# zqqqqz2000/MixGRPO

Hardware: AMD Instinct MI355X
Metric: GRPO train-step images/sec, FLUX.1-dev 1024^2 (higher is better)
Workload: dtype bf16

## Files before the change

mixgrpo_amd/csrc/small.hip:

```cpp
#include "../../include/mixgrpo_hip.h"
#include "common.h"

namespace {

__global__ void __launch_bounds__(256) skinny_linear_kernel(const bf16_raw* __restrict__ x, long ldx,
                                                            const bf16_raw* __restrict__ W, long ldw,
                                                            const bf16_raw* __restrict__ bias,
                                                            bf16_raw* __restrict__ out, long ldo, int Bn, int N, int K) {
  __shared__ f32x4 red[3][64];
  const int lane = threadIdx.x & 63, w = threadIdx.x >> 6;
  const int n0 = blockIdx.x * 16;
  const int fr = lane & 15, fq = lane >> 4;
  int nrow = n0 + fr;
  if (nrow >= N) nrow = N - 1;
  int brow = fr < Bn ? fr : Bn - 1;
  const int kchunk = ((K / 32 + 3) / 4) * 32;
  const int kbeg = min(w * kchunk, K), kend = min(kbeg + kchunk, K);
  const bf16_raw* wp = W + (long)nrow * ldw + fq * 8;
  const bf16_raw* xp = x + (long)brow * ldx + fq * 8;
  f32x4 acc = {0.f, 0.f, 0.f, 0.f};
  int k = kbeg;
  for (; k + 128 <= kend; k += 128) {
    s16x8 a0 = *reinterpret_cast<const s16x8*>(wp + k), a1 = *reinterpret_cast<const s16x8*>(wp + k + 32);
    s16x8 a2 = *reinterpret_cast<const s16x8*>(wp + k + 64), a3 = *reinterpret_cast<const s16x8*>(wp + k + 96);
    s16x8 b0 = *reinterpret_cast<const s16x8*>(xp + k), b1 = *reinterpret_cast<const s16x8*>(xp + k + 32);
    s16x8 b2 = *reinterpret_cast<const s16x8*>(xp + k + 64), b3 = *reinterpret_cast<const s16x8*>(xp + k + 96);
    acc = __builtin_amdgcn_mfma_f32_16x16x32_bf16(a0, b0, acc, 0, 0, 0);
    acc = __builtin_amdgcn_mfma_f32_16x16x32_bf16(a1, b1, acc, 0, 0, 0);
    acc = __builtin_amdgcn_mfma_f32_16x16x32_bf16(a2, b2, acc, 0, 0, 0);
    acc = __builtin_amdgcn_mfma_f32_16x16x32_bf16(a3, b3, acc, 0, 0, 0);
  }
  for (; k < kend; k += 32) {
    s16x8 a0 = *reinterpret_cast<const s16x8*>(wp + k);
    s16x8 b0 = *reinterpret_cast<const s16x8*>(xp + k);
    acc = __builtin_amdgcn_mfma_f32_16x16x32_bf16(a0, b0, acc, 0, 0, 0);
  }
  if (w > 0) red[w - 1][lane] = acc;
  __syncthreads();
  if (w > 0) return;
#pragma unroll
  for (int i = 0; i < 3; ++i) {
    const f32x4 o = red[i][lane];
    acc[0] += o[0]; acc[1] += o[1]; acc[2] += o[2]; acc[3] += o[3];
  }
  if (fr < Bn) {
#pragma unroll
    for (int r = 0; r < 4; ++r) {
      const int n = n0 + 4 * fq + r;
      if (n < N) {
        float v = acc[r];
        if (bias) v += bf2f(bias[n]);
        out[(long)fr * ldo + n] = f2bf(v);
      }
    }
  }
}

__global__ void __launch_bounds__(256) skinny_wgrad_kernel(const bf16_raw* __restrict__ dout, long ldd,
                                                           const bf16_raw* __restrict__ x, long ldx,
                                                           float* __restrict__ dW, long ldw, float* __restrict__ dbias,
                                                           int Bn, int N, int K) {
  const int n = blockIdx.y;
  float dn[16];
  float sb = 0.f;
#pragma unroll
  for (int b = 0; b < 16; ++b) {
    dn[b] = b < Bn ? bf2f(dout[(long)b * ldd + n]) : 0.f;
    sb += dn[b];
  }
  if (dbias && blockIdx.x == 0 && threadIdx.x == 0) dbias[n] += sb;
  for (int k = (blockIdx.x * 256 + threadIdx.x) * 4; k < K; k += gridDim.x * 256 * 4) {
    float4 g = *reinterpret_cast<float4*>(dW + (long)n * ldw + k);
    for (int b = 0; b < Bn; ++b) {
      const uint2 u = *reinterpret_cast<const uint2*>(x + (long)b * ldx + k);
      g.x += dn[b] * bf2f(u.x & 0xffff); g.y += dn[b] * bf2f(u.x >> 16);
      g.z += dn[b] * bf2f(u.y & 0xffff); g.w += dn[b] * bf2f(u.y >> 16);
    }
    *reinterpret_cast<float4*>(dW + (long)n * ldw + k) = g;
  }
}

constexpr int SD_G = 128;
__global__ void __launch_bounds__(256) skinny_dgrad_kernel(const bf16_raw* __restrict__ dout, long ldd,
                                                           const bf16_raw* __restrict__ W, long ldw, float* __restrict__ part,
                                                           int Bn, int N, int K) {
  extern __shared__ float dsh[];
  const int g = blockIdx.y;
  const int nrows = (N - g + SD_G - 1) / SD_G;
  for (int id = threadIdx.x; id < nrows * 8; id += 256) {
    const int i = id >> 3, b = id & 7;
    dsh[id] = b < Bn ? bf2f(dout[(long)b * ldd + g + (long)i * SD_G]) : 0.f;
  }
  __syncthreads();
  const int c = (blockIdx.x * 256 + threadIdx.x) * 8;
  if (c >= K) return;
  float acc[8][8];
#pragma unroll
  for (int b = 0; b < 8; ++b)
#pragma unroll
    for (int e = 0; e < 8; ++e) acc[b][e] = 0.f;
  const bf16_raw* wp = W + (long)g * ldw + c;
  const long step = (long)SD_G * ldw;
  int i = 0;
  for (; i + 4 <= nrows; i += 4) {
    uint4 u[4];
// ... 84 lines not shown
    a.x = bf2f(u.x & 0xffff) * scale; a.y = bf2f(u.x >> 16) * scale; a.z = bf2f(u.y & 0xffff) * scale; a.w = bf2f(u.y >> 16) * scale;
    b.x = bf2f(u.z & 0xffff) * scale; b.y = bf2f(u.z >> 16) * scale; b.z = bf2f(u.w & 0xffff) * scale; b.w = bf2f(u.w >> 16) * scale;
    *reinterpret_cast<float4*>(y + i) = a;
    *reinterpret_cast<float4*>(y + i + 4) = b;
  }
}

constexpr int GR_ROWS = 64;
__global__ void __launch_bounds__(256) gate_bwd_kernel(const bf16_raw* __restrict__ dout, long ldd, long d_rpb,
                                                       long d_bstride, const bf16_raw* __restrict__ y, long ldy,
                                                       const bf16_raw* __restrict__ gate, long gate_ld,
                                                       bf16_raw* __restrict__ dy, long lddy, float* __restrict__ part,
                                                       long rows_per_batch, int D, int blocks_per_batch) {
  const long b = blockIdx.y / blocks_per_batch;
  const long r0 = (long)(blockIdx.y % blocks_per_batch) * GR_ROWS;
  const int c = (blockIdx.x * 256 + threadIdx.x) * 2;
  if (c >= D) return;
  const uint32_t gu = *reinterpret_cast<const uint32_t*>(gate + b * gate_ld + c);
  const float g0 = bf2f(gu & 0xffff), g1 = bf2f(gu >> 16);
  float a0 = 0.f, a1 = 0.f;
  const long rend = min(r0 + (long)GR_ROWS, rows_per_batch);
  for (long r = r0; r < rend; ++r) {
    const long m = b * rows_per_batch + r;
    const uint32_t du = *reinterpret_cast<const uint32_t*>(dout + b * d_bstride + r * ldd + c);
    const uint32_t yu = *reinterpret_cast<const uint32_t*>(y + m * ldy + c);
    const float d0 = bf2f(du & 0xffff), d1 = bf2f(du >> 16);
    a0 += d0 * bf2f(yu & 0xffff);
    a1 += d1 * bf2f(yu >> 16);
    *reinterpret_cast<uint32_t*>(dy + m * lddy + c) = (uint32_t)f2bf(g0 * d0) | ((uint32_t)f2bf(g1 * d1) << 16);
  }
  part[(long)blockIdx.y * D + c] = a0;
  part[(long)blockIdx.y * D + c + 1] = a1;
}

__global__ void __launch_bounds__(256) gate_bwd_finish_kernel(const float* __restrict__ part, bf16_raw* __restrict__ dgate,
                                                              long gate_ld, int D, int blocks_per_batch) {
  __shared__ float red[4][64];
  const int b = blockIdx.y;
  const int cx = threadIdx.x & 63, ky = threadIdx.x >> 6;
  const int c = blockIdx.x * 64 + cx;
  float s = 0.f;
  if (c < D)
    for (int k = ky; k < blocks_per_batch; k += 4) s += part[((long)b * blocks_per_batch + k) * D + c];
  red[ky][cx] = s;
  __syncthreads();
  if (ky == 0 && c < D) dgate[(long)b * gate_ld + c] = f2bf((red[0][cx] + red[1][cx]) + (red[2][cx] + red[3][cx]));
}

}

extern "C" int mgx_skinny_linear(const uint16_t* x, long ldx, const uint16_t* W, long ldw, const uint16_t* bias,
                                 uint16_t* out, long ldo, int Bn, int N, int K, void* stream) {
  MGX_REQUIRE(x && W && out, "null operand");
  MGX_REQUIRE(Bn >= 1 && Bn <= 16, "skinny linear handles 1..16 rows");
  MGX_REQUIRE(K % 32 == 0 && ldx % 8 == 0 && ldw % 8 == 0, "K must be a multiple of 32 with 16-byte aligned rows");
  skinny_linear_kernel<<<cdiv(N, 16), 256, 0, (hipStream_t)stream>>>(x, ldx, W, ldw, bias, out, ldo, Bn, N, K);
  MGX_CHECK_LAUNCH();
  return MGX_OK;
}

extern "C" int mgx_skinny_wgrad(const uint16_t* dout, long ldd, const uint16_t* x, long ldx, float* dW, long ldw,
                                float* dbias, int Bn, int N, int K, void* stream) {
  MGX_REQUIRE(dout && x && dW, "null operand");
  MGX_REQUIRE(Bn >= 1 && Bn <= 16, "skinny wgrad handles 1..16 rows");
  MGX_REQUIRE(K % 4 == 0 && ldx % 4 == 0 && ldw % 4 == 0, "K must be a multiple of 4");
  int gx = cdiv(K, 1024);
  skinny_wgrad_kernel<<<dim3(gx, N), 256, 0, (hipStream_t)stream>>>(dout, ldd, x, ldx, dW, ldw, dbias, Bn, N, K);
  MGX_CHECK_LAUNCH();
  return MGX_OK;
}

extern "C" long mgx_skinny_dgrad_workspace(int Bn, int K) { return (long)SD_G * (Bn < 8 ? Bn : 8) * K; }

extern "C" int mgx_skinny_dgrad(const uint16_t* dout, long ldd, const uint16_t* W, long ldw, uint16_t* dx, long lddx,
                                float* ws, int Bn, int N, int K, int accumulate, void* stream) {
  MGX_REQUIRE(dout && W && dx && ws, "null operand");
  MGX_REQUIRE(Bn >= 1 && Bn <= 8, "skinny dgrad handles 1..8 rows per call");
  MGX_REQUIRE(N >= SD_G && K % 8 == 0 && ldw % 8 == 0 && ((uintptr_t)W % 16 == 0), "weight rows must be 16-byte addressable");
  hipStream_t st = (hipStream_t)stream;
  const size_t lds = (size_t)cdiv(N, SD_G) * 8 * sizeof(float);
  MGX_REQUIRE(lds <= 65536, "too many weight rows");
  skinny_dgrad_kernel<<<dim3(cdiv(K, 2048), SD_G), 256, lds, st>>>(dout, ldd, W, ldw, ws, Bn, N, K);
  skinny_dgrad_finish_kernel<<<cdiv((long)Bn * K, 256), 256, 0, st>>>(ws, dx, lddx, Bn, K, accumulate);
  MGX_CHECK_LAUNCH();
  return MGX_OK;
}

extern "C" int mgx_ew_bf16(const uint16_t* a, const uint16_t* b, uint16_t* y, long n, int op, void* stream) {
  MGX_REQUIRE(a && y && n > 0 && op >= 0 && op <= 3, "bad argument");
  MGX_REQUIRE(op == 0 || op == 3 || b, "binary op needs b");
  int nb = cdiv(n, 256);
  if (nb > 2048) nb = 2048;
  ew_kernel<<<nb, 256, 0, (hipStream_t)stream>>>(a, b, y, n, op);
  MGX_CHECK_LAUNCH();
  return MGX_OK;
}

extern "C" int mgx_sincos_embed(const float* t, uint16_t* out, int Bn, void* stream) {
  MGX_REQUIRE(t && out && Bn > 0, "bad argument");
  sincos_embed_kernel<<<Bn, 128, 0, (hipStream_t)stream>>>(t, out, Bn);
  MGX_CHECK_LAUNCH();
  return MGX_OK;
}

extern "C" int mgx_cast_f32_bf16(const float* x, uint16_t* y, long n, void* stream) {
  MGX_REQUIRE(x && y && n > 0 && n % 4 == 0, "bad argument");
  int nb = cdiv(n, 1024);
  if (nb > 4096) nb = 4096;
  cast_f32_bf16_kernel<<<nb, 256, 0, (hipStream_t)stream>>>(x, y, n);
// ... 32 lines not shown
```

mixgrpo_amd/flux.py:

```python
import json
import math
import os
from dataclasses import asdict, dataclass
from typing import Dict, List, Tuple

import torch

from . import ops
from ._lib import MgxError
from .ops import BF16, F32, Rows, EPI_BIAS, EPI_BIAS_GELU, EPI_BIAS_GATE_RES


@dataclass
class FluxConfig:
    patch_size: int = 1
    in_channels: int = 64
    num_layers: int = 19
    num_single_layers: int = 38
    attention_head_dim: int = 128
    num_attention_heads: int = 24
    joint_attention_dim: int = 4096
    pooled_projection_dim: int = 768
    guidance_embeds: bool = True
    axes_dims_rope: Tuple[int, int, int] = (16, 56, 56)
# ... 166 lines not shown
        self.out = e(B, N, cfg.patch_size * cfg.patch_size * cfg.in_channels)
        self.lse = e(B, H, S, dtype=F32)
        self.train = None
        self._f8 = None
        self._f8_bwd = None
        self._dims = (H, hd)

    def fp8_bwd_workspace(self):
        if self._f8_bwd is None:
            H, _ = self._dims
            dev = self.X.device
            self._f8_bwd = (torch.empty(ops.attn_bwd_fp8_workspace(self.B, H, self.S, self.Sp), dtype=torch.uint8, device=dev),
                            torch.empty(4 * self.B * H, dtype=F32, device=dev))
        return self._f8_bwd

    def fp8_operands(self):
        if self._f8 is None:
            H, hd = self._dims
            u8 = lambda *shape: torch.empty(*shape, dtype=torch.uint8, device=self.X.device)
            self._f8 = (u8(self.B, H, self.S, hd), u8(self.B, H, self.S, hd), u8(self.B, H, hd, self.Sp),
                        torch.empty(3 * self.B * H, dtype=F32, device=self.X.device))
        return self._f8

    def view(self, B, kv_len=None):
        return self if B == self.B and kv_len is None else _WorkView(self, B, kv_len)


class _WorkView:

    def __init__(self, base, B, kv_len=None):
        assert B <= base.B
        self.base, self.B, self.L, self.N, self.S, self.Sp, self.kv_len = base, B, base.L, base.N, base.S, base.Sp, kv_len
        M = B * base.S
        self.X, self.Q, self.K, self.Vt, self.O, self.cat = (t[:B] for t in (base.X, base.Q, base.K, base.Vt, base.O, base.cat))
        self.nrm, self.qkv, self.hid = base.nrm[:M], base.qkv[:M], base.hid[:M]
        self.in16, self.out, self.lse = base.in16[:B * base.N], base.out[:B], base.lse[:B]

    def fp8_operands(self):
        q8, k8, v8t, amax = self.base.fp8_operands()
        return q8[:self.B], k8[:self.B], v8t[:self.B], amax

    def fp8_bwd_workspace(self):
        return self.base.fp8_bwd_workspace()

    @property
    def train(self):
        return self.base.train

    @train.setter
    def train(self, v):
        self.base.train = v


class FluxTransformer2DModel(torch.nn.Module):

    def __init__(self, config: FluxConfig = None, device="cuda", attention_dtype="bf16", **cfg_kwargs):
        super().__init__()
        if attention_dtype not in ("bf16", "fp8"):
            raise ValueError(f"attention_dtype {attention_dtype!r} is not supported (bf16 | fp8)")
        self.attention_dtype = attention_dtype
        self.cfg = config or FluxConfig(**cfg_kwargs)
        self.config = self.cfg.to_dict()
        dev = torch.device(device)
        if dev.type != "cuda":
            raise MgxError("FluxTransformer2DModel (mixgrpo_amd) runs on an MI355X only; there is no CPU path")
        self.store = ParamStore(self.cfg, dev)
        self.flat_param = torch.nn.Parameter(self.store.w32, requires_grad=True)
        self._work: Dict[Tuple[int, int], _Work] = {}
        self._rope_cache = {}
        self.recompute = True
        self.last_route = None
        self.padded_kv_calls = 0
        self.last_train_route = None
        self.padded_kv_train_calls = 0

    def state_dict(self, *args, **kwargs):
        return {k: self.store.view(self.store.w32, k) for k in self.store.index}

    def load_state_dict(self, sd, strict=True):
        missing = [k for k in self.store.index if k not in sd]
        unexpected = [k for k in sd if k not in self.store.index]
        if strict and (missing or unexpected):
            raise RuntimeError(f"load_state_dict: missing {missing[:5]} unexpected {unexpected[:5]}")
        with torch.no_grad():
            for k, v in sd.items():
                if k in self.store.index:
                    self.store.view(self.store.w32, k).copy_(v.to(F32))
        self.store.sync_bf16()
        return missing, unexpected

    def init_synthetic(self, seed=0, std=0.02, bias_std=0.0):
        self.store.init_synthetic(seed, std, bias_std)
        return self

    def W(self, name):
        return self.store.view(self.store.w16, name)

    def W32(self, name):
        return self.store.view(self.store.w32, name)

    def clip_grad_norm_(self, max_norm):
        g = self.store.ensure_grad()
        nsq = torch.zeros(1, dtype=F32, device=g.device)
        ops.sqnorm(g, nsq)
        total = nsq.sqrt()
        coef = torch.clamp(max_norm / (total + 1e-6), max=1.0)
# ... 106 lines not shown
            ops.ew(h1, None, a1, 0)
            h2 = torch.empty_like(h1)
            ops.skinny_linear(a1, self.W(f"time_text_embed.{name}.linear_2.weight"),
                              self.W(f"time_text_embed.{name}.linear_2.bias"), h2, d, d)
            if keep is not None:
                keep[name] = (x, h1, a1)
            return h2

        te = torch.empty(B, 256, dtype=BF16, device=dev)
        ops.sincos_embed(t, te)
        temb = mlp("timestep_embedder", te, 256)
        if self.cfg.guidance_embeds:
            ge = torch.empty(B, 256, dtype=BF16, device=dev)
            ops.sincos_embed(gd, ge)
            gemb = mlp("guidance_embedder", ge, 256)
            t2 = torch.empty_like(temb)
            ops.ew(temb, gemb, t2, 2)
            temb = t2
        pe = mlp("text_embedder", pooled.to(BF16).contiguous(), self.cfg.pooled_projection_dim)
        t3 = torch.empty_like(temb)
        ops.ew(temb, pe, t3, 2)
        st = torch.empty_like(t3)
        ops.ew(t3, None, st, 0)
        return t3, st

    def _stream_rows(self, t, w, which, width):
        if which == "txt":
            return Rows(t, w.B * w.L, width, w.L, w.S * width)
        return Rows(t[0, w.L:], w.B * w.N, width, w.N, w.S * width)

    def _streams(self, w):
        streams = (("txt", "norm1_context", ("add_q_proj", "add_k_proj", "add_v_proj"), "norm_added_q", "norm_added_k",
                    "to_add_out", "ff_context", w.L, 0),
                   ("img", "norm1", ("to_q", "to_k", "to_v"), "norm_q", "norm_k", "to_out.0", "ff", w.N, w.L))
        return streams, {"txt": slice(0, w.B * w.L), "img": slice(w.B * w.L, w.B * w.S)}

    def _double_block(self, i, w, st, cos, sin, pl, mods_in=None):
        cfg, d, H = self.cfg, self.cfg.dim, self.cfg.num_attention_heads
        p = f"transformer_blocks.{i}"
        B = w.B
        dev = self.store.device
        mods = {}
        streams, sl = self._streams(w)
        W16, fused = self.W, self.store.fused
        if pl.restore is not None:
            w.X.copy_(pl.restore)
        for name, norm, qkvn, nq, nk, outn, ffn, rows, s0 in streams:
            if mods_in is not None:
                m = mods_in[name]
            else:
                m = torch.empty(B, 6 * d, dtype=BF16, device=dev)
                ops.skinny_linear(st, W16(f"{p}.{norm}.linear.weight"), W16(f"{p}.{norm}.linear.bias"), m, 6 * d, d)
            mods[name] = m
            ops.ln_modulate(self._stream_rows(pl.x_in, w, name, d), m[:, 0:d], m[:, d:2 * d], 6 * d, pl.nrm1[sl[name]], d)
        if pl.fused_qkv:
            for name, _, qkvn, nq, nk, _, _, rows, s0 in streams:
                self._qkv_nograd(pl.nrm1[sl[name]], f"{p}.attn.{qkvn[0]}", pl.qkv[sl[name]], w, rows, s0,
                                 self.W32(f"{p}.attn.{nq}.weight"), self.W32(f"{p}.attn.{nk}.weight"), cos, sin)
        else:
            for name, _, qkvn, *_ in (streams if pl.run_qkv else ()):
                ops.gemm(Rows.of(pl.nrm1[sl[name]]), fused(self.store.w16, f"{p}.attn.{qkvn[0]}.weight", 3 * d),
                         fused(self.store.w16, f"{p}.attn.{qkvn[0]}.bias", 3 * d), Rows.of(pl.qkv[sl[name]]), 3 * d, d)
            for name, norm, qkvn, nq, nk, outn, ffn, rows, s0 in streams:
                ops.qk_norm_rope(pl.qkv[sl[name]], self.W32(f"{p}.attn.{nq}.weight"), self.W32(f"{p}.attn.{nk}.weight"), cos, sin,
                                 w.Q, w.K, w.Vt, B, H, w.S, w.Sp, rows, s0, V=pl.V, Qt=pl.Qt, Kt=pl.Kt, q_scale=self.q_scale())
        if pl.run_attn:
            self._attn(w, pl.O, pl.lse, d, w.S * d)
        part = lambda t, name: None if t is None else t[sl[name]]
        if pl.run_out:
            for name, _, _, _, _, outn, *_ in streams:
                ops.gemm(self._stream_rows(pl.O, w, name, d), W16(f"{p}.attn.{outn}.weight"), W16(f"{p}.attn.{outn}.bias"),
                         self._stream_rows(w.X, w, name, d), d, d, EPI_BIAS_GATE_RES, gate=mods[name][:, 2 * d:3 * d],
                         gate_ld=6 * d, aux=part(pl.y_attn, name))
            if pl.x_mid is not None:
                pl.x_mid.copy_(w.X)
        x_mid = w.X if pl.run_out else pl.x_mid
        for name in ("txt", "img"):
            m = mods[name]
            ops.ln_modulate(self._stream_rows(x_mid, w, name, d), m[:, 3 * d:4 * d], m[:, 4 * d:5 * d], 6 * d, pl.nrm2[sl[name]], d)
        for name, _, _, _, _, _, ffn, *_ in (streams if pl.run_ff else ()):
            ops.gemm(Rows.of(pl.nrm2[sl[name]]), W16(f"{p}.{ffn}.net.0.proj.weight"), W16(f"{p}.{ffn}.net.0.proj.bias"),
                     Rows.of(w.hid[sl[name]]), 4 * d, d, EPI_BIAS_GELU, aux=part(pl.hid_pre, name))
        for name, _, _, _, _, _, ffn, *_ in (streams if pl.run_out else ()):
            ops.gemm(Rows.of(w.hid[sl[name]]), W16(f"{p}.{ffn}.net.2.weight"), W16(f"{p}.{ffn}.net.2.bias"),
                     self._stream_rows(w.X, w, name, d), d, 4 * d, EPI_BIAS_GATE_RES, gate=mods[name][:, 5 * d:6 * d],
                     gate_ld=6 * d, aux=part(pl.y_ff, name))
        return mods

    def _single_block(self, i, w, st, cos, sin, pl, mod_in=None):
        cfg, d, H = self.cfg, self.cfg.dim, self.cfg.num_attention_heads
        p = f"single_transformer_blocks.{i}"
        B, S = w.B, w.S
        M = B * S
        if pl.restore is not None:
            w.X.copy_(pl.restore)
        if mod_in is not None:
            m = mod_in
        else:
            m = torch.empty(B, 3 * d, dtype=BF16, device=self.store.device)
            ops.skinny_linear(st, self.W(f"{p}.norm.linear.weight"), self.W(f"{p}.norm.linear.bias"), m, 3 * d, d)
        Xa = Rows(pl.x_in, M, d, S, S * d)
        ops.ln_modulate(Xa, m[:, 0:d], m[:, d:2 * d], 3 * d, pl.nrm1, d)
        wq, wk = self.W32(f"{p}.attn.norm_q.weight"), self.W32(f"{p}.attn.norm_k.weight")
        if pl.fused_qkv:
            self._qkv_nograd(pl.nrm1, f"{p}.attn.to_q", pl.qkv, w, S, 0, wq, wk, cos, sin)
        elif pl.run_qkv:
            ops.gemm(Rows.of(pl.nrm1), self.store.fused(self.store.w16, f"{p}.attn.to_q.weight", 3 * d),
                     self.store.fused(self.store.w16, f"{p}.attn.to_q.bias", 3 * d), Rows.of(pl.qkv), 3 * d, d)
        cat2 = w.cat.view(M, 5 * d)
        if pl.run_ff:
            ops.gemm(Rows.of(pl.nrm1), self.W(f"{p}.proj_mlp.weight"), self.W(f"{p}.proj_mlp.bias"),
                     Rows(cat2[0, d:], M, 5 * d), 4 * d, d, EPI_BIAS_GELU, aux=pl.hid_pre)
        if not pl.fused_qkv:
            ops.qk_norm_rope(pl.qkv, wq, wk, cos, sin, w.Q, w.K, w.Vt, B, H, S, w.Sp, S, 0, V=pl.V, Qt=pl.Qt, Kt=pl.Kt,
                             q_scale=self.q_scale())
        if pl.run_attn:
            self._attn(w, pl.O, pl.lse, pl.ldo, S * pl.ldo)
            if pl.O_keep is not None:
                pl.O_keep.copy_(w.cat[:, :, :d])
        elif not pl.lean:
            w.cat[:, :, :d].copy_(pl.O_keep)
        if pl.run_out:
            ops.gemm(Rows.of(cat2), self.W(f"{p}.proj_out.weight"), self.W(f"{p}.proj_out.bias"), Xa, d, 5 * d,
                     EPI_BIAS_GATE_RES, gate=m[:, 2 * d:3 * d], gate_ld=3 * d, aux=pl.y_attn)
        return m

    def _embed(self, w, hidden_states, encoder_hidden_states):
        d = self.cfg.dim
        B, N, L = w.B, w.N, w.L
        hs = hidden_states.detach()
        if hs.dtype == BF16:
            w.in16.copy_(hs.reshape(B * N, -1))
        else:
            ops.cast_bf16(hs.to(F32).contiguous().view(-1), w.in16.view(-1))
        ops.gemm(Rows.of(w.in16), self.W("x_embedder.weight"), self.W("x_embedder.bias"),
                 self._stream_rows(w.X, w, "img", d), d, self.cfg.in_channels)
        ehs = encoder_hidden_states.detach().to(BF16).contiguous()
        ops.gemm(Rows.of(ehs.view(B * L, -1)), self.W("context_embedder.weight"), self.W("context_embedder.bias"),
                 self._stream_rows(w.X, w, "txt", d), d, self.cfg.joint_attention_dim)
        return ehs

    def _head(self, w, st):
        d = self.cfg.dim
        B, N = w.B, w.N
        e = torch.empty(B, 2 * d, dtype=BF16, device=self.store.device)
        ops.skinny_linear(st, self.W("norm_out.linear.weight"), self.W("norm_out.linear.bias"), e, 2 * d, d)
        nrm = w.nrm[:B * N]
        ops.ln_modulate(self._stream_rows(w.X, w, "img", d), e[:, d:2 * d], e[:, 0:d], 2 * d, nrm, d)
        cout = self.cfg.patch_size * self.cfg.patch_size * self.cfg.in_channels
        out = torch.empty(B, N, cout, dtype=BF16, device=self.store.device)
        ops.gemm(Rows.of(nrm), self.W("proj_out.weight"), self.W("proj_out.bias"), Rows.of(out.view(B * N, cout)), cout, d)
        return out, e

    def forward(self, hidden_states, encoder_hidden_states, timestep, guidance, txt_ids, pooled_projections, img_ids,
                joint_attention_kwargs=None, return_dict=False):
        if torch.is_grad_enabled() and self.training and self.flat_param.requires_grad:
            from .flux_backward import FluxFunction
            out = FluxFunction.apply(self.flat_param, self, hidden_states, encoder_hidden_states, timestep, guidance,
                                     txt_ids, pooled_projections, img_ids)
            return (out,)
        with torch.no_grad():
            out = self._forward_nograd(hidden_states, encoder_hidden_states, timestep, guidance, txt_ids,
                                       pooled_projections, img_ids)
        return (out,)

    def _pad_kv_rows(self, B, L, N):
        S = L + N
        if not ops.ATTN_PAD_KV or S % 256 == 0 or not ops.Q_PRESCALE or self.attention_dtype != "bf16":
            return None
        d, H = self.cfg.dim, self.cfg.num_attention_heads
        Sa = (S + 255) // 256 * 256
        if not all(ops.attn_fwd_kv_path(B, H, Sa, S, ld, Sa * ld) == 1 for ld in (d, 5 * d)):
            return None
        return Sa - L

    def _pad_kv_rows_train(self, B, L, N):
        N_pad = self._pad_kv_rows(B, L, N)
        if N_pad is None:
            return None
        d, H = self.cfg.dim, self.cfg.num_attention_heads
        Sa = L + N_pad
        if not all(ops.attn_bwd_kv_path(B, H, Sa, L + N, ld, Sa * ld) == 1 for ld in (d, 5 * d)):
            return None
        return N_pad

    def _padded_inputs(self, hidden_states, img_ids, N_pad):
        B, N, C = hidden_states.shape
        hs = hidden_states.new_zeros(B, N_pad, C)
        hs[:, :N] = hidden_states
        key = (id(img_ids), img_ids._version, tuple(img_ids.shape), N_pad)
        hit = self._rope_cache.get("pad_ids")
        if hit is None or hit[0] != key:
            ids = torch.cat([img_ids, img_ids.new_zeros(N_pad - N, img_ids.shape[1])], dim=0)
            hit = (key, ids, img_ids)
            self._rope_cache["pad_ids"] = hit
        return hs, hit[1]

    def _forward_nograd(self, hidden_states, encoder_hidden_states, timestep, guidance, txt_ids, pooled_projections,
                        img_ids, collect=None):
        B, N, _ = hidden_states.shape
        L = encoder_hidden_states.shape[1]
        N_pad = self._pad_kv_rows(B, L, N) if collect is None else None
        if N_pad is not None:
            hs, ids = self._padded_inputs(hidden_states, img_ids, N_pad)
            out = self._forward_nograd_on(self._workspace(B, L, N_pad, kv_len=L + N), hs, encoder_hidden_states, timestep, guidance,
                                          txt_ids, pooled_projections, ids, None)
            self.last_route = "padded_kv"
            self.padded_kv_calls += 1
            return out[:, :N].contiguous()
        self.last_route = "plain"
        return self._forward_nograd_on(self._workspace(B, L, N), hidden_states, encoder_hidden_states, timestep, guidance, txt_ids,
                                       pooled_projections, img_ids, collect)

    def _forward_nograd_on(self, w, hidden_states, encoder_hidden_states, timestep, guidance, txt_ids, pooled_projections,
                           img_ids, collect):
        from .flux_backward import _BlockPlan
        B, L = w.B, w.L
        double, single = _BlockPlan(w, True), _BlockPlan(w, False)
        self._embed(w, hidden_states, encoder_hidden_states)
        temb, st = self._temb(B, timestep.to(self.store.device), guidance, pooled_projections)
        cos, sin = self._rope(txt_ids, img_ids)
        if collect is not None:
            collect.update(temb=temb.clone(), x_embed=w.X[:, L:].clone(), ctx_embed=w.X[:, :L].clone())
        for i in range(self.cfg.num_layers):
            self._double_block(i, w, st, cos, sin, double)
            if collect is not None:
                collect[f"double{i}_h"] = w.X[:, L:].clone()
                collect[f"double{i}_c"] = w.X[:, :L].clone()
        for i in range(self.cfg.num_single_layers):
            self._single_block(i, w, st, cos, sin, single)
            if collect is not None:
                collect[f"single{i}_x"] = w.X.clone()
        out, _ = self._head(w, st)
        return out

    def save_pretrained(self, save_dir):
        from safetensors.torch import save_file
        os.makedirs(save_dir, exist_ok=True)
        sd = {k: v.detach().cpu().contiguous() for k, v in self.state_dict().items()}
        save_file(sd, os.path.join(save_dir, "diffusion_pytorch_model.safetensors"))
        cfg = dict(self.config)
        cfg.pop("dtype", None)
        with open(os.path.join(save_dir, "config.json"), "w") as f:
            json.dump(cfg, f, indent=4)

    @classmethod
    def from_pretrained(cls, path, device="cuda", subfolder=None, torch_dtype=None):
        from safetensors.torch import load_file
        if subfolder and os.path.isdir(os.path.join(path, subfolder)):
            path = os.path.join(path, subfolder)
        with open(os.path.join(path, "config.json")) as f:
            raw = json.load(f)
        keys = {f.name for f in FluxConfig.__dataclass_fields__.values()}
        cfg = FluxConfig(**{k: (tuple(v) if k == "axes_dims_rope" else v) for k, v in raw.items() if k in keys})
        m = cls(cfg, device=device)
        index = os.path.join(path, "diffusion_pytorch_model.safetensors.index.json")
        if os.path.exists(index):
            with open(index) as f:
                shards = sorted(set(json.load(f)["weight_map"].values()))
            sd = {}
            for shard in shards:
                sd.update(load_file(os.path.join(path, shard)))
        else:
            sd = load_file(os.path.join(path, "diffusion_pytorch_model.safetensors"))
        m.load_state_dict(sd)
        return m
```

mixgrpo_amd/ops.py:

```python
import os
from dataclasses import dataclass

import torch

from ._lib import check, lib, ptr, stream

EPI_BIAS, EPI_BIAS_GELU, EPI_BIAS_GATE_RES, EPI_F32_ACC, EPI_DGELU = 0, 1, 2, 3, 4
BF16 = torch.bfloat16
F32 = torch.float32


@dataclass
class Rows:
    t: torch.Tensor
    M: int
    ld: int
    rpb: int = 1 << 40
    bstride: int = 0

    @staticmethod
    def of(t):
        cols = t.shape[-1]
        return Rows(t, t.numel() // cols, cols)

# ... 143 lines not shown


ATTN_PAD_KV = os.environ.get("MGX_ATTN_PAD_KV", "0") != "0"


def attn_fwd_log2_kv(Q2, K, Vt, O_ptr_tensor, lse, B, H, Sa, kv_len, ldo, o_bstride):
    return _try(lib().mgx_attn_fwd_log2_kv, ptr(Q2), ptr(K), ptr(Vt), O_ptr_tensor.data_ptr(), ptr(lse), B, H, Sa, kv_len, ldo, o_bstride,
                stream())


def attn_fwd_kv_path(B, H, Sa, kv_len, ldo, o_bstride):
    return lib().mgx_attn_fwd_kv_path(B, H, Sa, kv_len, ldo, o_bstride)


def attn_bwd_path(B, H, S, Sp, ldo, o_bstride):
    r = lib().mgx_attn_bwd_path(B, H, S, Sp, ldo, o_bstride)
    check(min(r, 0))
    return r


def attn_fp8_quantize(Q, K, Vt, Q8, K8, V8t, amax, B, H, S, Sp):
    check(lib().mgx_attn_fp8_quantize(ptr(Q), ptr(K), ptr(Vt), ptr(Q8), ptr(K8), ptr(V8t), ptr(amax), B, H, S, Sp,
                                      stream()))


def attn_fwd_fp8(Q8, K8, V8t, amax, O_ptr_tensor, lse, B, H, S, Sp, ldo, o_bstride, scale):
    check(lib().mgx_attn_fwd_fp8(ptr(Q8), ptr(K8), ptr(V8t), ptr(amax), O_ptr_tensor.data_ptr(), ptr(lse), B, H, S, Sp,
                                 ldo, o_bstride, scale, stream()))


ATTN_FP8_BWD = os.environ.get("MGX_ATTN_FP8_BWD", "0") != "0"


def attn_bwd_fp8_workspace(B, H, S, Sp):
    n = lib().mgx_attn_bwd_fp8_workspace(B, H, S, Sp)
    if n < 0:
        raise ValueError(f"attn_bwd_fp8_workspace: bad sizes B {B} H {H} S {S} Sp {Sp}")
    return n


def attn_bwd_fp8_layout(B, H, S, Sp):
    rb, tb = (B * H * S * 128 + 255) // 256 * 256, B * H * 128 * Sp
    out = {n: (i * rb, (B, H, S, 128)) for i, n in enumerate(("Q8", "K8", "V8", "dO8"))}
    out.update({n: (4 * rb + i * tb, (B, H, 128, Sp)) for i, n in enumerate(("Q8t", "K8t", "dO8t"))})
    return out


def attn_bwd_fp8(Q, K, V, Qt, Kt, O, dO, lse, delta, dOt, dQ, dK, dV, ws, amax, B, H, S, Sp, ldo, o_bstride, scale):
    check(lib().mgx_attn_bwd_fp8(ptr(Q), ptr(K), ptr(V), ptr(Qt), ptr(Kt), O.data_ptr(), dO.data_ptr(), ptr(lse), ptr(delta),
                                 ptr(dOt), ptr(dQ), ptr(dK), ptr(dV), ptr(ws), ptr(amax), B, H, S, Sp, ldo, o_bstride, scale,
                                 ws.numel(), stream()))


def skinny_linear(x, W, bias, out, N, K):
    Bn = x.shape[0]
    for b0 in range(0, Bn, 16):
        nb = min(16, Bn - b0)
        check(lib().mgx_skinny_linear(x[b0:].data_ptr(), x.stride(0), ptr(W), K, ptr(bias), out[b0:].data_ptr(),
                                      out.stride(0), nb, N, K, stream()))


def skinny_wgrad(dout, x, dW, dbias, N, K):
    Bn = x.shape[0]
    for b0 in range(0, Bn, 16):
        nb = min(16, Bn - b0)
        check(lib().mgx_skinny_wgrad(dout[b0:].data_ptr(), dout.stride(0), x[b0:].data_ptr(), x.stride(0), ptr(dW), K,
                                     ptr(dbias), nb, N, K, stream()))


def skinny_dgrad(dout, W, dx, N, K, accumulate=True):
    Bn = dout.shape[0]
    for b0 in range(0, Bn, 8):
        nb = min(8, Bn - b0)
        ws = scratch("skinny_dgrad", lib().mgx_skinny_dgrad_workspace(nb, K), F32, dout.device)
        check(lib().mgx_skinny_dgrad(dout[b0:].data_ptr(), dout.stride(0), ptr(W), K, dx[b0:].data_ptr(), dx.stride(0),
                                     ptr(ws), nb, N, K, 1 if accumulate else 0, stream()))


def ew(a, b, y, op):
    check(lib().mgx_ew_bf16(ptr(a), ptr(b), ptr(y), a.numel(), op, stream()))


def sincos_embed(t, out):
    check(lib().mgx_sincos_embed(ptr(t), ptr(out), t.numel(), stream()))


def cast_bf16(x, y):
    check(lib().mgx_cast_f32_bf16(ptr(x), ptr(y), x.numel(), stream()))


def gelu_rows(x, ldx, y, ldy, M, N):
    check(lib().mgx_gelu_bf16(ptr(x), ldx, ptr(y), ldy, M, N, stream()))


def cast_f32(x, y, scale=1.0):
    check(lib().mgx_cast_bf16_f32(ptr(x), ptr(y), x.numel(), float(scale), stream()))


def gate_bwd(dout: Rows, y, gate, gate_ld, dy, dgate, batches, rows_per_batch, D):
    ws = scratch("gate_bwd", lib().mgx_gate_bwd_workspace(batches, rows_per_batch, D), F32, y.device)
    check(lib().mgx_gate_bwd(ptr(dout.t), dout.ld, dout.bstride, ptr(y), D, gate.data_ptr(), gate_ld, ptr(dy), D,
                             dgate.data_ptr(), ptr(ws), batches, rows_per_batch, D, stream()))


def sqnorm(g, out, beta=0.0):
    ws = scratch("sqnorm", lib().mgx_sqnorm_workspace(), torch.float64, g.device)
    check(lib().mgx_sqnorm_f32(ptr(g), g.numel(), ptr(ws), ptr(out), beta, stream()))


def adamw_step(w, w16, g, m, v, lr, beta1, beta2, eps, wd, step, gnorm_sq, max_norm, grad_scale=1.0):
# ... 48 lines not shown
```

mixgrpo_amd/sampling_utils.py:

```python
import ctypes as C
import math
from dataclasses import dataclass
from typing import List, Optional

import numpy as np
import torch

from . import _lib
from ._lib import DanceCoeffs, DpmCoeffs, FlowCoeffs, check, lib, logp_workspace, ptr, stream

SCALAR_ROUNDING = "cpu"
_F32 = torch.float32
_BF16 = torch.bfloat16
_LOG_SQRT_2PI = torch.log(torch.sqrt(2 * torch.as_tensor(math.pi)))


def sd3_time_shift(shift, t):
    return (shift * t) / (1 + (shift - 1) * t)


def _host(sigmas):
    return sigmas if not sigmas.is_cuda else sigmas.detach().cpu()


# ... 297 lines not shown

def dpm_step(args, model_output, sample, step_index, timesteps, sigmas, dpm_state=None, generator=None,
             variance_noise=None, sde_solver=False, x_out=None):
    step_index = int(step_index)
    n_ts = len(timesteps)
    final = step_index == n_ts - 1
    second = step_index == n_ts - 2 and n_ts < 15
    dev = model_output.device
    x = _as(sample, _F32)
    v = _as(model_output, _BF16)
    B, n = _flat(x)
    if dpm_state:
        lo = dpm_state.lower_order_nums
        if args.dpm_solver_order == 1 or lo < 1 or final:
            order = 1
        elif args.dpm_solver_order == 2 or lo < 2 or second:
            order = 2
        else:
            order = 3
        hist = dpm_state.model_outputs
        m1 = hist[-1] if order >= 2 else None
        m2 = hist[-2] if order >= 3 else None
    else:
        order, m1, m2 = 1, None, None
    noise = None
    if sde_solver:
        noise = (torch.randn(x.shape, generator=generator, device=dev, dtype=_F32) if variance_noise is None
                 else _as(variance_noise.to(dev), _F32))
    k = dpm_coeffs(args.dpm_algorithm_type, args.dpm_solver_type, order, sigmas, step_index, sde_solver)
    out = x_out if x_out is not None else torch.empty_like(x)
    if sde_solver and not dpm_state and model_output.requires_grad and torch.is_grad_enabled():
        return _DpmSdeLogp.apply(model_output, x, noise, k, _u(_host(sigmas).to(_F32)[step_index]), out)
    x0 = torch.empty_like(x)
    logp = torch.empty(B, dtype=_F32, device=dev)
    check(lib().mgx_dpm_step_fwd(ptr(x), ptr(v), ptr(m1), ptr(m2), ptr(noise), ptr(out), ptr(x0), ptr(logp),
                                 ptr(logp_workspace(B, n, dev)), B, n, C.byref(k), stream()))
    if dpm_state is not None:
        dpm_state.update(x0)
        dpm_state.update_lower_order()
    return out, x0, logp


def flash_schedule(sigma_schedule, determistic, ratio, shift):
    sg = _host(sigma_schedule)
    n = sg.size(0)
    sde_idx = [i for i, d in enumerate(determistic) if not d]
    last = sde_idx[-1]
    num_post = int(max((n - 1 - last) * ratio, 1))
    t0 = torch.linspace(1, 0, n)[last + 1].item()
    post = sd3_time_shift(shift, torch.linspace(t0, 0, num_post))
    return torch.cat([sg[:last + 1], post], dim=0), last


def run_sample_step(args, z, progress_bar, sigma_schedule, transformer, encoder_hidden_states, pooled_prompt_embeds,
                    text_ids, image_ids, grpo_sample, determistic, noises=None, shared_rows=False):
    dev = z.device
    noises = iter(noises) if noises is not None else None
    sig = _host(sigma_schedule).to(_F32)
    use_dpm = "dpmsolver" in args.dpm_algorithm_type
    post = use_dpm and args.dpm_apply_strategy == "post"
    state = DPMState(order=args.dpm_solver_order) if use_dpm else None
    last_sde = None
    if post:
        assert args.sample_strategy == "progressive", "post strategy is only supported for progressive sampling"
        sig, last_sde = flash_schedule(sig, determistic, args.dpm_post_compress_ratio, args.shift)
        progress_bar = range(sig.size(0) - 1)
    steps = sig.size(0) - 1
    B = encoder_hidden_states.shape[0]
    buf = torch.empty((steps + 1,) + tuple(z.shape), dtype=_F32, device=dev)
    buf[0].copy_(z)
    logps = torch.empty(steps, z.shape[0], dtype=_F32, device=dev)
    guidance = torch.tensor([3.5], device=dev, dtype=_BF16)
    txt_ids = text_ids.repeat(encoder_hidden_states.shape[1], 1)
    x0 = None
    n_run = 0
    first_noisy = steps
    if shared_rows and B > 1:
        for j in range(steps):
            in_flow = (not use_dpm) or (post and j <= last_sde)
            if (in_flow or not post) and not determistic[j]:
                first_noisy = j
                break
    else:
        first_noisy = -1
    ehs_all, pooled_all = encoder_hidden_states, pooled_prompt_embeds
    for i in progress_bar:
        one = shared_rows and B > 1 and i <= first_noisy
        solve_one = shared_rows and B > 1 and i < first_noisy
        encoder_hidden_states = ehs_all[:1] if one else ehs_all
        pooled_prompt_embeds = pooled_all[:1] if one else pooled_all
        timestep_value = int(sig[i] * 1000)
        timestep = torch.full([1 if one else B], float(np.float32(timestep_value) / np.float32(1000)), device=dev,
                              dtype=_F32)
        transformer.eval()
        with torch.autocast("cuda", torch.bfloat16):
            pred = transformer(hidden_states=z[:1] if one else z, encoder_hidden_states=encoder_hidden_states,
                               timestep=timestep, guidance=guidance, txt_ids=txt_ids,
                               pooled_projections=pooled_prompt_embeds, img_ids=image_ids, joint_attention_kwargs=None,
                               return_dict=False)[0]
        if one and not solve_one:
            pred = pred.expand(B, -1, -1).contiguous()
            if state is not None:
                state.model_outputs = [None if m is None else m.expand(B, -1, -1).contiguous()
                                       for m in state.model_outputs]
        zf = buf[i]
        nxt = buf[i + 1]
        if solve_one:
            zf, nxt = zf[:1], nxt[:1]
        keep_x0 = args.drop_last_sample and i == steps - 1
        if (not use_dpm) or (post and i <= last_sde):
            if args.flow_grpo_sampling:
                nz = next(noises) if noises is not None else None
                if nz is not None and solve_one:
                    nz = nz[:1]
                _, x0_i, lp, _, _ = flow_grpo_step(pred, zf, args.eta, sig, i, None, determistic=determistic[i],
                                                   noise=nz, prev_out=nxt, want_x0=keep_x0 or post, want_mean=False)
                if post:
                    state.update(x0_i)
                    state.update_lower_order()
            else:
                sde = not determistic[i]
                nz = next(noises) if (noises is not None and sde) else None
                _, x0_i, lp = dance_grpo_step(pred, zf, args.eta, sig, i, None, True, sde, noise=nz, prev_out=nxt)
        elif post:
            _, x0_i, lp = dpm_step(args, pred, zf, i, sig[:-1], sig, dpm_state=state, sde_solver=False, x_out=nxt)
        else:
            sde = not determistic[i]
            nz = next(noises) if (noises is not None and sde) else None
            _, x0_i, lp = dpm_step(args, pred, zf, i, sig[:-1], sig, dpm_state=state,
                                   generator=None if nz is not None else torch.Generator(device=dev),
                                   variance_noise=nz, sde_solver=sde, x_out=nxt)
        if solve_one:
            buf[i + 1][1:].copy_(nxt.expand(B - 1, -1, -1))
            nxt = buf[i + 1]
            lp = lp.expand(B)
            if x0_i is not None:
                x0_i = x0_i.expand(B, -1, -1)
        x0 = x0_i
        z = nxt
        logps[i].copy_(lp)
        n_run += 1
    latents = x0 if args.drop_last_sample else z
    return z, latents, buf.transpose(0, 1), logps.transpose(0, 1)
```

Baseline: 0.4389.

## Precompute per-rollout conditioning modulation table batched across all sampling steps

Before sampling, computes timestep embeddings and all adaLN modulation projections for every step (and batch row) in one batched pass, then feeds row views of the table into each forward. This way each modulation weight matrix is streamed once per rollout instead of once per step. The skinny linear kernel gains a two-tile template to handle up to 32 rows per weight pass, and ln_modulate and gate calls now take strides from the tensor so expanded or sliced views work. This adds memory for the table and relies on timesteps known ahead, with broadcast views where the prompt is shared.

```diff
diff --git a/mixgrpo_amd/cond_table.py b/mixgrpo_amd/cond_table.py
--- /dev/null
+++ b/mixgrpo_amd/cond_table.py
@@ -0,0 +1,33 @@
+from dataclasses import dataclass
+from typing import List, Optional, Tuple
+
+ROWS_PER_PASS = 32
+MAX_ROWS = 256
+
+
+def weight_passes(rows):
+    return -(-rows // ROWS_PER_PASS)
+
+
+@dataclass
+class RolloutPlan:
+    rows: List[Tuple[int, int]]
+    forward_rows: list
+
+    def passes(self):
+        return weight_passes(len(self.rows))
+
+
+def rollout_plan(steps, B, shared_prompt) -> Optional[RolloutPlan]:
+    if steps < 1 or B < 1:
+        return None
+    if shared_prompt:
+        rows = [(i, 0) for i in range(steps)]
+        fwd = list(range(steps))
+    else:
+        rows = [(i, b) for i in range(steps) for b in range(B)]
+        fwd = [(i * B, (i + 1) * B) for i in range(steps)]
+    plan = RolloutPlan(rows, fwd)
+    if len(rows) > MAX_ROWS or plan.passes() >= steps * weight_passes(B):
+        return None
+    return plan
diff --git a/mixgrpo_amd/csrc/small.hip b/mixgrpo_amd/csrc/small.hip
--- a/mixgrpo_amd/csrc/small.hip
+++ b/mixgrpo_amd/csrc/small.hip
@@ -3,54 +3,73 @@
 
 namespace {
 
+template <int TILES>
 __global__ void __launch_bounds__(256) skinny_linear_kernel(const bf16_raw* __restrict__ x, long ldx,
                                                             const bf16_raw* __restrict__ W, long ldw,
                                                             const bf16_raw* __restrict__ bias,
                                                             bf16_raw* __restrict__ out, long ldo, int Bn, int N, int K) {
-  __shared__ f32x4 red[3][64];
+  __shared__ f32x4 red[3][TILES][64];
   const int lane = threadIdx.x & 63, w = threadIdx.x >> 6;
   const int n0 = blockIdx.x * 16;
   const int fr = lane & 15, fq = lane >> 4;
   int nrow = n0 + fr;
   if (nrow >= N) nrow = N - 1;
-  int brow = fr < Bn ? fr : Bn - 1;
   const int kchunk = ((K / 32 + 3) / 4) * 32;
   const int kbeg = min(w * kchunk, K), kend = min(kbeg + kchunk, K);
   const bf16_raw* wp = W + (long)nrow * ldw + fq * 8;
-  const bf16_raw* xp = x + (long)brow * ldx + fq * 8;
-  f32x4 acc = {0.f, 0.f, 0.f, 0.f};
+  const bf16_raw* xp[TILES];
+  f32x4 acc[TILES];
+#pragma unroll
+  for (int t = 0; t < TILES; ++t) {
+    const int brow = 16 * t + fr < Bn ? 16 * t + fr : Bn - 1;
+    xp[t] = x + (long)brow * ldx + fq * 8;
+    acc[t] = f32x4{0.f, 0.f, 0.f, 0.f};
+  }
   int k = kbeg;
   for (; k + 128 <= kend; k += 128) {
     s16x8 a0 = *reinterpret_cast<const s16x8*>(wp + k), a1 = *reinterpret_cast<const s16x8*>(wp + k + 32);
     s16x8 a2 = *reinterpret_cast<const s16x8*>(wp + k + 64), a3 = *reinterpret_cast<const s16x8*>(wp + k + 96);
-    s16x8 b0 = *reinterpret_cast<const s16x8*>(xp + k), b1 = *reinterpret_cast<const s16x8*>(xp + k + 32);
-    s16x8 b2 = *reinterpret_cast<const s16x8*>(xp + k + 64), b3 = *reinterpret_cast<const s16x8*>(xp + k + 96);
-    acc = __builtin_amdgcn_mfma_f32_16x16x32_bf16(a0, b0, acc, 0, 0, 0);
-    acc = __builtin_amdgcn_mfma_f32_16x16x32_bf16(a1, b1, acc, 0, 0, 0);
-    acc = __builtin_amdgcn_mfma_f32_16x16x32_bf16(a2, b2, acc, 0, 0, 0);
-    acc = __builtin_amdgcn_mfma_f32_16x16x32_bf16(a3, b3, acc, 0, 0, 0);
+#pragma unroll
+    for (int t = 0; t < TILES; ++t) {
+      s16x8 b0 = *reinterpret_cast<const s16x8*>(xp[t] + k), b1 = *reinterpret_cast<const s16x8*>(xp[t] + k + 32);
+      s16x8 b2 = *reinterpret_cast<const s16x8*>(xp[t] + k + 64), b3 = *reinterpret_cast<const s16x8*>(xp[t] + k + 96);
+      acc[t] = __builtin_amdgcn_mfma_f32_16x16x32_bf16(a0, b0, acc[t], 0, 0, 0);
+      acc[t] = __builtin_amdgcn_mfma_f32_16x16x32_bf16(a1, b1, acc[t], 0, 0, 0);
+      acc[t] = __builtin_amdgcn_mfma_f32_16x16x32_bf16(a2, b2, acc[t], 0, 0, 0);
+      acc[t] = __builtin_amdgcn_mfma_f32_16x16x32_bf16(a3, b3, acc[t], 0, 0, 0);
+    }
   }
   for (; k < kend; k += 32) {
     s16x8 a0 = *reinterpret_cast<const s16x8*>(wp + k);
-    s16x8 b0 = *reinterpret_cast<const s16x8*>(xp + k);
-    acc = __builtin_amdgcn_mfma_f32_16x16x32_bf16(a0, b0, acc, 0, 0, 0);
-  }
-  if (w > 0) red[w - 1][lane] = acc;
+#pragma unroll
+    for (int t = 0; t < TILES; ++t) {
+      s16x8 b0 = *reinterpret_cast<const s16x8*>(xp[t] + k);
+      acc[t] = __builtin_amdgcn_mfma_f32_16x16x32_bf16(a0, b0, acc[t], 0, 0, 0);
+    }
+  }
+  if (w > 0) {
+#pragma unroll
+    for (int t = 0; t < TILES; ++t) red[w - 1][t][lane] = acc[t];
+  }
   __syncthreads();
   if (w > 0) return;
 #pragma unroll
-  for (int i = 0; i < 3; ++i) {
-    const f32x4 o = red[i][lane];
-    acc[0] += o[0]; acc[1] += o[1]; acc[2] += o[2]; acc[3] += o[3];
-  }
-  if (fr < Bn) {
-#pragma unroll
-    for (int r = 0; r < 4; ++r) {
-      const int n = n0 + 4 * fq + r;
-      if (n < N) {
-        float v = acc[r];
-        if (bias) v += bf2f(bias[n]);
-        out[(long)fr * ldo + n] = f2bf(v);
+  for (int t = 0; t < TILES; ++t) {
+#pragma unroll
+    for (int i = 0; i < 3; ++i) {
+      const f32x4 o = red[i][t][lane];
+      acc[t][0] += o[0]; acc[t][1] += o[1]; acc[t][2] += o[2]; acc[t][3] += o[3];
+    }
+    const int b = 16 * t + fr;
+    if (b < Bn) {
+#pragma unroll
+      for (int r = 0; r < 4; ++r) {
+        const int n = n0 + 4 * fq + r;
+        if (n < N) {
+          float v = acc[t][r];
+          if (bias) v += bf2f(bias[n]);
+          out[(long)b * ldo + n] = f2bf(v);
+        }
       }
     }
   }
@@ -241,9 +260,12 @@
 extern "C" int mgx_skinny_linear(const uint16_t* x, long ldx, const uint16_t* W, long ldw, const uint16_t* bias,
                                  uint16_t* out, long ldo, int Bn, int N, int K, void* stream) {
   MGX_REQUIRE(x && W && out, "null operand");
-  MGX_REQUIRE(Bn >= 1 && Bn <= 16, "skinny linear handles 1..16 rows");
-  MGX_REQUIRE(K % 32 == 0 && ldx % 8 == 0 && ldw % 8 == 0, "K must be a multiple of 32 with 16-byte aligned rows");
-  skinny_linear_kernel<<<cdiv(N, 16), 256, 0, (hipStream_t)stream>>>(x, ldx, W, ldw, bias, out, ldo, Bn, N, K);
+  MGX_REQUIRE(Bn >= 1 && Bn <= 32, "skinny linear handles 1..32 rows");
+  MGX_REQUIRE(N >= 1 && K % 32 == 0 && ldx % 8 == 0 && ldw % 8 == 0, "K must be a multiple of 32 with 16-byte aligned rows");
+  if (Bn <= 16)
+    skinny_linear_kernel<1><<<cdiv(N, 16), 256, 0, (hipStream_t)stream>>>(x, ldx, W, ldw, bias, out, ldo, Bn, N, K);
+  else
+    skinny_linear_kernel<2><<<cdiv(N, 16), 256, 0, (hipStream_t)stream>>>(x, ldx, W, ldw, bias, out, ldo, Bn, N, K);
   MGX_CHECK_LAUNCH();
   return MGX_OK;
 }
diff --git a/mixgrpo_amd/flux.py b/mixgrpo_amd/flux.py
--- a/mixgrpo_amd/flux.py
+++ b/mixgrpo_amd/flux.py
@@ -242,6 +242,21 @@
         self.base.train = v
 
 
+class CondTable:
+
+    def __init__(self, temb, st, double, single, e):
+        self.temb, self.st, self.double, self.single, self.e = temb, st, double, single, e
+        self.rows = st.shape[0]
+
+    @staticmethod
+    def view(t, rows, B):
+        if isinstance(rows, int):
+            return t[rows:rows + 1].expand(B, -1)
+        first, stop = rows
+        assert stop - first == B, f"conditioning rows {rows} for a forward at batch {B}"
+        return t[first:stop]
+
+
 class FluxTransformer2DModel(torch.nn.Module):
 
     def __init__(self, config: FluxConfig = None, device="cuda", attention_dtype="bf16", **cfg_kwargs):
@@ -454,7 +469,7 @@
                 m = torch.empty(B, 6 * d, dtype=BF16, device=dev)
                 ops.skinny_linear(st, W16(f"{p}.{norm}.linear.weight"), W16(f"{p}.{norm}.linear.bias"), m, 6 * d, d)
             mods[name] = m
-            ops.ln_modulate(self._stream_rows(pl.x_in, w, name, d), m[:, 0:d], m[:, d:2 * d], 6 * d, pl.nrm1[sl[name]], d)
+            ops.ln_modulate(self._stream_rows(pl.x_in, w, name, d), m[:, 0:d], m[:, d:2 * d], m.stride(0), pl.nrm1[sl[name]], d)
         if pl.fused_qkv:
             for name, _, qkvn, nq, nk, _, _, rows, s0 in streams:
                 self._qkv_nograd(pl.nrm1[sl[name]], f"{p}.attn.{qkvn[0]}", pl.qkv[sl[name]], w, rows, s0,
@@ -473,20 +488,20 @@
             for name, _, _, _, _, outn, *_ in streams:
                 ops.gemm(self._stream_rows(pl.O, w, name, d), W16(f"{p}.attn.{outn}.weight"), W16(f"{p}.attn.{outn}.bias"),
                          self._stream_rows(w.X, w, name, d), d, d, EPI_BIAS_GATE_RES, gate=mods[name][:, 2 * d:3 * d],
-                         gate_ld=6 * d, aux=part(pl.y_attn, name))
+                         gate_ld=mods[name].stride(0), aux=part(pl.y_attn, name))
             if pl.x_mid is not None:
                 pl.x_mid.copy_(w.X)
         x_mid = w.X if pl.run_out else pl.x_mid
         for name in ("txt", "img"):
             m = mods[name]
-            ops.ln_modulate(self._stream_rows(x_mid, w, name, d), m[:, 3 * d:4 * d], m[:, 4 * d:5 * d], 6 * d, pl.nrm2[sl[name]], d)
+            ops.ln_modulate(self._stream_rows(x_mid, w, name, d), m[:, 3 * d:4 * d], m[:, 4 * d:5 * d], m.stride(0), pl.nrm2[sl[name]], d)
         for name, _, _, _, _, _, ffn, *_ in (streams if pl.run_ff else ()):
             ops.gemm(Rows.of(pl.nrm2[sl[name]]), W16(f"{p}.{ffn}.net.0.proj.weight"), W16(f"{p}.{ffn}.net.0.proj.bias"),
                      Rows.of(w.hid[sl[name]]), 4 * d, d, EPI_BIAS_GELU, aux=part(pl.hid_pre, name))
         for name, _, _, _, _, _, ffn, *_ in (streams if pl.run_out else ()):
             ops.gemm(Rows.of(w.hid[sl[name]]), W16(f"{p}.{ffn}.net.2.weight"), W16(f"{p}.{ffn}.net.2.bias"),
                      self._stream_rows(w.X, w, name, d), d, 4 * d, EPI_BIAS_GATE_RES, gate=mods[name][:, 5 * d:6 * d],
-                     gate_ld=6 * d, aux=part(pl.y_ff, name))
+                     gate_ld=mods[name].stride(0), aux=part(pl.y_ff, name))
         return mods
 
     def _single_block(self, i, w, st, cos, sin, pl, mod_in=None):
@@ -502,7 +517,7 @@
             m = torch.empty(B, 3 * d, dtype=BF16, device=self.store.device)
             ops.skinny_linear(st, self.W(f"{p}.norm.linear.weight"), self.W(f"{p}.norm.linear.bias"), m, 3 * d, d)
         Xa = Rows(pl.x_in, M, d, S, S * d)
-        ops.ln_modulate(Xa, m[:, 0:d], m[:, d:2 * d], 3 * d, pl.nrm1, d)
+        ops.ln_modulate(Xa, m[:, 0:d], m[:, d:2 * d], m.stride(0), pl.nrm1, d)
         wq, wk = self.W32(f"{p}.attn.norm_q.weight"), self.W32(f"{p}.attn.norm_k.weight")
         if pl.fused_qkv:
             self._qkv_nograd(pl.nrm1, f"{p}.attn.to_q", pl.qkv, w, S, 0, wq, wk, cos, sin)
@@ -524,7 +539,7 @@
             w.cat[:, :, :d].copy_(pl.O_keep)
         if pl.run_out:
             ops.gemm(Rows.of(cat2), self.W(f"{p}.proj_out.weight"), self.W(f"{p}.proj_out.bias"), Xa, d, 5 * d,
-                     EPI_BIAS_GATE_RES, gate=m[:, 2 * d:3 * d], gate_ld=3 * d, aux=pl.y_attn)
+                     EPI_BIAS_GATE_RES, gate=m[:, 2 * d:3 * d], gate_ld=m.stride(0), aux=pl.y_attn)
         return m
 
     def _embed(self, w, hidden_states, encoder_hidden_states):
@@ -542,20 +557,22 @@
                  self._stream_rows(w.X, w, "txt", d), d, self.cfg.joint_attention_dim)
         return ehs
 
-    def _head(self, w, st):
+    def _head(self, w, st, e_in=None):
         d = self.cfg.dim
         B, N = w.B, w.N
-        e = torch.empty(B, 2 * d, dtype=BF16, device=self.store.device)
-        ops.skinny_linear(st, self.W("norm_out.linear.weight"), self.W("norm_out.linear.bias"), e, 2 * d, d)
+        e = e_in
+        if e is None:
+            e = torch.empty(B, 2 * d, dtype=BF16, device=self.store.device)
+            ops.skinny_linear(st, self.W("norm_out.linear.weight"), self.W("norm_out.linear.bias"), e, 2 * d, d)
         nrm = w.nrm[:B * N]
-        ops.ln_modulate(self._stream_rows(w.X, w, "img", d), e[:, d:2 * d], e[:, 0:d], 2 * d, nrm, d)
+        ops.ln_modulate(self._stream_rows(w.X, w, "img", d), e[:, d:2 * d], e[:, 0:d], e.stride(0), nrm, d)
         cout = self.cfg.patch_size * self.cfg.patch_size * self.cfg.in_channels
         out = torch.empty(B, N, cout, dtype=BF16, device=self.store.device)
         ops.gemm(Rows.of(nrm), self.W("proj_out.weight"), self.W("proj_out.bias"), Rows.of(out.view(B * N, cout)), cout, d)
         return out, e
 
     def forward(self, hidden_states, encoder_hidden_states, timestep, guidance, txt_ids, pooled_projections, img_ids,
-                joint_attention_kwargs=None, return_dict=False):
+                joint_attention_kwargs=None, return_dict=False, cond=None):
         if torch.is_grad_enabled() and self.training and self.flat_param.requires_grad:
             from .flux_backward import FluxFunction
             out = FluxFunction.apply(self.flat_param, self, hidden_states, encoder_hidden_states, timestep, guidance,
@@ -563,7 +580,7 @@
             return (out,)
         with torch.no_grad():
             out = self._forward_nograd(hidden_states, encoder_hidden_states, timestep, guidance, txt_ids,
-                                       pooled_projections, img_ids)
+                                       pooled_projections, img_ids, cond=cond)
         return (out,)
 
     def _pad_kv_rows(self, B, L, N):
@@ -599,42 +616,66 @@
         return hs, hit[1]
 
     def _forward_nograd(self, hidden_states, encoder_hidden_states, timestep, guidance, txt_ids, pooled_projections,
-                        img_ids, collect=None):
+                        img_ids, collect=None, cond=None):
         B, N, _ = hidden_states.shape
         L = encoder_hidden_states.shape[1]
         N_pad = self._pad_kv_rows(B, L, N) if collect is None else None
         if N_pad is not None:
             hs, ids = self._padded_inputs(hidden_states, img_ids, N_pad)
             out = self._forward_nograd_on(self._workspace(B, L, N_pad, kv_len=L + N), hs, encoder_hidden_states, timestep, guidance,
-                                          txt_ids, pooled_projections, ids, None)
+                                          txt_ids, pooled_projections, ids, None, cond)
             self.last_route = "padded_kv"
             self.padded_kv_calls += 1
             return out[:, :N].contiguous()
         self.last_route = "plain"
         return self._forward_nograd_on(self._workspace(B, L, N), hidden_states, encoder_hidden_states, timestep, guidance, txt_ids,
-                                       pooled_projections, img_ids, collect)
+                                       pooled_projections, img_ids, collect, cond)
 
     def _forward_nograd_on(self, w, hidden_states, encoder_hidden_states, timestep, guidance, txt_ids, pooled_projections,
-                           img_ids, collect):
+                           img_ids, collect, cond=None):
         from .flux_backward import _BlockPlan
         B, L = w.B, w.L
         double, single = _BlockPlan(w, True), _BlockPlan(w, False)
         self._embed(w, hidden_states, encoder_hidden_states)
-        temb, st = self._temb(B, timestep.to(self.store.device), guidance, pooled_projections)
+        if cond is not None:
+            tab, rows = cond
+            row = lambda t: CondTable.view(t, rows, B)
+            temb, st = row(tab.temb), None
+            dmods = [{k: row(v) for k, v in m.items()} for m in tab.double]
+            smods, e_in = [row(m) for m in tab.single], row(tab.e)
+        else:
+            temb, st = self._temb(B, timestep.to(self.store.device), guidance, pooled_projections)
+            dmods, smods, e_in = [None] * self.cfg.num_layers, [None] * self.cfg.num_single_layers, None
         cos, sin = self._rope(txt_ids, img_ids)
         if collect is not None:
             collect.update(temb=temb.clone(), x_embed=w.X[:, L:].clone(), ctx_embed=w.X[:, :L].clone())
         for i in range(self.cfg.num_layers):
-            self._double_block(i, w, st, cos, sin, double)
+            self._double_block(i, w, st, cos, sin, double, mods_in=dmods[i])
             if collect is not None:
                 collect[f"double{i}_h"] = w.X[:, L:].clone()
                 collect[f"double{i}_c"] = w.X[:, :L].clone()
         for i in range(self.cfg.num_single_layers):
-            self._single_block(i, w, st, cos, sin, single)
+            self._single_block(i, w, st, cos, sin, single, mod_in=smods[i])
             if collect is not None:
                 collect[f"single{i}_x"] = w.X.clone()
-        out, _ = self._head(w, st)
+        out, _ = self._head(w, st, e_in)
         return out
+
+    def cond_table(self, timestep, guidance, pooled_projections):
+        d, dev = self.cfg.dim, self.store.device
+        R = timestep.shape[0]
+        with torch.no_grad():
+            temb, st = self._temb(R, timestep.to(dev), guidance, pooled_projections)
+
+            def lin(prefix, n):
+                m = torch.empty(R, n * d, dtype=BF16, device=dev)
+                ops.skinny_linear(st, self.W(f"{prefix}.linear.weight"), self.W(f"{prefix}.linear.bias"), m, n * d, d)
+                return m
+
+            double = [{"txt": lin(f"transformer_blocks.{i}.norm1_context", 6), "img": lin(f"transformer_blocks.{i}.norm1", 6)}
+                      for i in range(self.cfg.num_layers)]
+            single = [lin(f"single_transformer_blocks.{i}.norm", 3) for i in range(self.cfg.num_single_layers)]
+            return CondTable(temb, st, double, single, lin("norm_out", 2))
 
     def save_pretrained(self, save_dir):
         from safetensors.torch import save_file
diff --git a/mixgrpo_amd/ops.py b/mixgrpo_amd/ops.py
--- a/mixgrpo_amd/ops.py
+++ b/mixgrpo_amd/ops.py
@@ -219,10 +219,14 @@
                                  ws.numel(), stream()))
 
 
+SKINNY_ROWS = 32
+COND_TABLE = os.environ.get("MGX_COND_TABLE", "1") != "0"
+
+
 def skinny_linear(x, W, bias, out, N, K):
     Bn = x.shape[0]
-    for b0 in range(0, Bn, 16):
-        nb = min(16, Bn - b0)
+    for b0 in range(0, Bn, SKINNY_ROWS):
+        nb = min(SKINNY_ROWS, Bn - b0)
         check(lib().mgx_skinny_linear(x[b0:].data_ptr(), x.stride(0), ptr(W), K, ptr(bias), out[b0:].data_ptr(),
                                       out.stride(0), nb, N, K, stream()))
 
diff --git a/mixgrpo_amd/sampling_utils.py b/mixgrpo_amd/sampling_utils.py
--- a/mixgrpo_amd/sampling_utils.py
+++ b/mixgrpo_amd/sampling_utils.py
@@ -373,6 +373,20 @@
     return torch.cat([sg[:last + 1], post], dim=0), last
 
 
+def _rollout_cond_table(transformer, t_host, guidance, pooled, B, shared_prompt, dev):
+    from . import ops
+    from .cond_table import rollout_plan
+    if not ops.COND_TABLE or not hasattr(transformer, "cond_table"):
+        return None
+    plan = rollout_plan(len(t_host), B, shared_prompt)
+    if plan is None:
+        return None
+    t = torch.tensor([t_host[i] for i, _ in plan.rows], dtype=_F32).to(dev)
+    pooled_rows = pooled[:1].expand(len(plan.rows), -1) if shared_prompt else pooled.repeat(len(t_host), 1)
+    with torch.autocast("cuda", torch.bfloat16):
+        return transformer.cond_table(t, guidance, pooled_rows), plan
+
+
 def run_sample_step(args, z, progress_bar, sigma_schedule, transformer, encoder_hidden_states, pooled_prompt_embeds,
                     text_ids, image_ids, grpo_sample, determistic, noises=None, shared_rows=False):
     dev = z.device
@@ -405,20 +419,21 @@
     else:
         first_noisy = -1
     ehs_all, pooled_all = encoder_hidden_states, pooled_prompt_embeds
+    t_host = [float(np.float32(int(sig[j] * 1000)) / np.float32(1000)) for j in range(steps)]
+    cond = _rollout_cond_table(transformer, t_host, guidance, pooled_all, B, shared_rows and B > 1, dev)
     for i in progress_bar:
         one = shared_rows and B > 1 and i <= first_noisy
         solve_one = shared_rows and B > 1 and i < first_noisy
         encoder_hidden_states = ehs_all[:1] if one else ehs_all
         pooled_prompt_embeds = pooled_all[:1] if one else pooled_all
-        timestep_value = int(sig[i] * 1000)
-        timestep = torch.full([1 if one else B], float(np.float32(timestep_value) / np.float32(1000)), device=dev,
-                              dtype=_F32)
+        timestep = torch.full([1 if one else B], t_host[i], device=dev, dtype=_F32)
         transformer.eval()
+        kw = {} if cond is None else {"cond": (cond[0], cond[1].forward_rows[i])}
         with torch.autocast("cuda", torch.bfloat16):
             pred = transformer(hidden_states=z[:1] if one else z, encoder_hidden_states=encoder_hidden_states,
                                timestep=timestep, guidance=guidance, txt_ids=txt_ids,
                                pooled_projections=pooled_prompt_embeds, img_ids=image_ids, joint_attention_kwargs=None,
-                               return_dict=False)[0]
+                               return_dict=False, **kw)[0]
         if one and not solve_one:
             pred = pred.expand(B, -1, -1).contiguous()
             if state is not None:
```

Measured after the change: 0.4402, median of 6. About the same (+0.3%).
